# hustvl/LSFA

Measured on AMD Instinct MI355X. Metric: frames/sec/GPU at 1000x600 key_interval=10 (whole-job frames/s), higher is better.
Workload: dtype f32

## Files before the change

### include/lsfa_hip.h

```cpp
#ifndef LSFA_HIP_H_
#define LSFA_HIP_H_

#include <stddef.h>
#include <stdint.h>

#ifdef __cplusplus
extern "C" {
#endif

#define LSFA_OK 0
#define LSFA_EINVAL (-1)
#define LSFA_EWORKSPACE (-2)
#define LSFA_ENOTSUP (-3)

const char* lsfa_last_error(void);
int lsfa_abi_version(void);

int lsfa_psroi_pool_fwd(const float* data, const float* rois,
                        int N, int C, int H, int W, int R,
                        float spatial_scale, int output_dim, int pooled_size, int group_size,
                        float* out, float* mapping_channel, void* stream);

int lsfa_rfcn_head_fwd(const float* cls_map, const float* box_map, const float* rois,
                       int N, int H, int W, int R, int ncls, int nbox,
// ... 76 lines not shown
                               double im_h, double im_w, double scale,
                               double score_thresh, double nms_thresh, int max_per_image,
                               double* dets, int* counts, int* keep_idx,
                               void* ws, size_t ws_bytes, void* stream);

int lsfa_rpn_softmax_split(const float* logits, int N, int H, int W, int ld, int A, float* cls_prob, float* bbox_pred, void* stream);

int lsfa_bbox_pred_clip(const float* rois, const float* deltas, int R, int nreg,
                        double im_h, double im_w, double scale, double* pred_boxes, void* stream);

int lsfa_deform_im2col(const float* data, const float* offset,
                       int N, int C, int H, int W, int kh, int kw,
                       int pad, int stride, int dilate, int deform_groups,
                       int Ho, int Wo, float* col, void* stream);

int lsfa_deform_im2col_cl(const float* data, const float* offset,
                          int N, int C, int H, int W, int kh, int kw,
                          int pad, int stride, int dilate, int deform_groups,
                          int Ho, int Wo, float* col, void* stream);
int lsfa_deform_im2col_cl_ld(const float* data, const float* offset, int offset_ld,
                             int N, int C, int H, int W, int kh, int kw,
                             int pad, int stride, int dilate, int deform_groups,
                             int Ho, int Wo, float* col, void* stream);

size_t lsfa_conv_nhwc_workspace_bytes(int N, int H, int W, int Cout, int kh, int kw, int stride, int pad, int dil);
int lsfa_conv_nhwc_fwd(const float* x, int N, int H, int W, int Cin, const float* w, const float* bias, int Cout,
                       int kh, int kw, int stride, int pad, int dil, int relu, float* y,
                       void* ws, size_t ws_bytes, void* stream);

int lsfa_conv_nhwc_fused_fwd(const float* x, int N, int H, int W, int Cin, const float* w, const float* bias, int Cout,
                             int kh, int kw, int stride, int pad, int dil, int relu, const float* residual, float* y,
                             float* y2, const float* scale2, const float* shift2,
                             void* ws, size_t ws_bytes, void* stream);

typedef struct lsfa_conv_desc {
  const float* x; int lda; int N, H, W, Cin;
  const void* wfrag; int pieces; int w_exp; const float* amax_in;
  const float* bias; int Cout, kh, kw, stride, pad_h, pad_w, dil;
  int act; int y_nchw; const float* residual; float* y; int ldy;
  float* y2; const float* scale2; const float* shift2;
  unsigned* amax_out; unsigned* status;
  int Ho, Wo, out_H, out_W, out_sy, out_sx;
  int prof_tag;
  int x_nchw;
  const float* in_scale;
  const float* in_shift;
  const float* w_scale;
} lsfa_conv_desc;
size_t lsfa_conv_weight_bytes(int Cout, int kh, int kw, int Cin, int pieces);
int lsfa_conv_weights(const float* w, int Cout, int kh, int kw, int Cin, int pieces, int w_exp, void* wfrag, void* stream);
int lsfa_conv_weights_pc(const float* w, int Cout, int kh, int kw, int Cin, const int* w_exp_pc, void* wfrag, void* stream);
size_t lsfa_conv_workspace_bytes(const lsfa_conv_desc* d);
int lsfa_conv_fwd(const lsfa_conv_desc* d, void* ws, size_t ws_bytes, void* stream);
int lsfa_amax_partial(const float* x, long long n, float* out256, void* stream);
#define LSFA_EOVERFLOW (-4)
int lsfa_status_check(unsigned* status_dev, void* stream);
int lsfa_conv_plan_override(int kernel, int nt, int st, int slices);
int lsfa_conv_order_override(int tile_order, int k_order);
int lsfa_conv_plan_query(const lsfa_conv_desc* d, int* out8);
size_t lsfa_deconv4x4s2_crop_workspace_bytes(int N, int Hi, int Wi, int Cin, int Cout, int Hc, int Wc, int pieces);
int lsfa_deconv4x4s2_crop_fwd(const float* x, int lda, int N, int Hi, int Wi, int Cin, const void* wfrag4, int pieces, int w_exp,
                              const float* amax_in, const float* bias, int Cout, int act, float* y, int ldy, int Hc, int Wc,
                              unsigned* amax_out, unsigned* status, void* ws, size_t ws_bytes, void* stream);

int lsfa_avgpool_nchw(const float* x, int N, int C, int H, int W, int k, float* y, void* stream);
int lsfa_avgpool_nchw_tbl(const float* const* x_table, int N, int C, int H, int W, int k, float* y, void* stream);
int lsfa_image_transform_u8(const unsigned char* im_hwc_bgr, int N, int H, int W, const double* pixel_means_bgr_host, double pixel_scale,
                            float* data_nchw, void* stream);
size_t lsfa_stem_weight_bytes(void);
int lsfa_stem_weights(const float* w_l, void* wfrag, void* stream);
int lsfa_stem_conv7x7s2(const float* x, int N, int H, int W, const float* in_scale, const float* in_shift,
                        const void* wfrag, const float* bias, float* y, void* stream);
int lsfa_maxpool3x3s2_nhwc(const float* x, int N, int H, int W, int C, float* y, float* y2, const float* scale2,
                           const float* shift2, unsigned* amax_out, void* stream);
int lsfa_stem_conv7x7s2_ex(const float* x, int N, int H, int W, const float* in_scale, const float* in_shift,
                           const void* wfrag, const float* bias, const float* accum, int act, float* y, unsigned* amax_out,
                           void* stream);
int lsfa_stem_conv7x7s2_tbl(const float* const* x_table, int N, int H, int W, const float* in_scale, const float* in_shift,
                            const void* wfrag, const float* bias, const float* accum, int act, float* y, unsigned* amax_out, void* stream);

int lsfa_head_conv3x3(const float* x, int lda, int N, int H, int W, int Cin, const float* w, const float* bias, int Cout,
                      float mul, float* y, int out_nchw, int ldy, int c0, void* stream);
int lsfa_upsample_flow(const float* in, int N, int Hi, int Wi, int C, const float* w, const float* bias, int Hc, int Wc,
                       float* out, int ldy, int c0, unsigned* amax_out, void* stream);
int lsfa_avgpool2_nhwc(const float* x, int N, int H, int W, int C, float* y, void* stream);
int lsfa_nchw_to_nhwc(const float* x, int N, int Ctot, int HW, int c0, int C, float* y, unsigned* amax_out, void* stream);

int lsfa_scale_shift_relu(const float* x, const float* scale, const float* shift,
                          int N, int C, int HW, int relu, float* y, void* stream);

int lsfa_scale_shift_leaky(const float* x, const float* scale, const float* shift,
                           int N, int C, int HW, float slope, float* y, void* stream);

int lsfa_scale_shift_relu_cl(const float* x, const float* scale, const float* shift,
                             long long rows, int C, int relu, float* y, void* stream);

size_t lsfa_mv_workspace_bytes(int width, int height);
int lsfa_mv_identity(int* accu, int width, int height, void* stream);
int lsfa_mv_accumulate(const int* mvs, int n_mvs, int max_block_area, const int* accu_old, int* accu_new,
                       int width, int height, void* ws, size_t ws_bytes, void* stream);
int lsfa_mv_field(const int* accu, int width, int height, int* mv, void* stream);
int lsfa_mv_residual(const unsigned char* bgr_cur, const unsigned char* bgr_ref, const int* accu,
                     int width, int height, int* res, void* stream);
int lsfa_transform_mv_res(const void* motion_vector, const void* res_diff, int flags, int H, int W, double im_scale, int h1, int w1,
                          int rcnn_stride, const double* pixel_means_bgr_host, double pixel_scale, float* out_mv, float* out_res,
                          int out_h, int out_w, void* stream);
// ... 52 lines not shown
```

### lsfa_amd/build.py

```python
import os
import subprocess
import sys
from concurrent.futures import ThreadPoolExecutor

HERE = os.path.dirname(os.path.abspath(__file__))
CSRC = os.path.join(HERE, "csrc")
INCLUDE = os.path.join(os.path.dirname(HERE), "include")
OBJ = os.path.join(HERE, "csrc", "_obj")
LIB = os.path.join(HERE, "liblsfa_hip.so")
SOURCES = ["runtime.hip", "warp.hip", "aggregate.hip", "psroi.hip", "nms.hip", "proposal.hip", "detpost.hip", "dcn.hip", "mv.hip", "me.hip", "me_segment.hip", "me_pyramid.hip", "yuv.hip", "conv.hip", "conv_exact.hip", "stem.hip", "flownet.hip", "rpn_head.hip", "fuse.hip"]
HIPCC = os.environ.get("HIPCC", "/opt/rocm/bin/hipcc")
FLAGS = ["--offload-arch=gfx950", "-O3", "-std=c++17", "-fPIC", "-ffp-contract=off", "-fno-fast-math",
         "-Wall", "-Wno-unused-function", "-I", INCLUDE, "-I", CSRC] + os.environ.get("LSFA_HIPCC_EXTRA", "-fno-slp-vectorize -fno-vectorize").split()


def _stale(target, deps):
    if not os.path.exists(target):
        return True
    t = os.path.getmtime(target)
    return any(os.path.getmtime(d) > t for d in deps)


def build_hip(force=False, verbose=False):
    os.makedirs(OBJ, exist_ok=True)
    headers = [os.path.join(CSRC, f) for f in os.listdir(CSRC) if f.endswith(".h")] + \
              [os.path.join(INCLUDE, "lsfa_hip.h")]
    jobs = []
    for src in SOURCES:
        s = os.path.join(CSRC, src)
        o = os.path.join(OBJ, src.replace(".hip", ".o"))
        if force or _stale(o, [s] + headers):
            jobs.append((s, o))

    def cc(job):
        s, o = job
        cmd = [HIPCC] + FLAGS + ["-c", s, "-o", o]
        if verbose:
            print(" ".join(cmd))
        r = subprocess.run(cmd, capture_output=True, text=True)
        if r.returncode != 0:
            raise RuntimeError("hipcc failed for %s:\n%s" % (s, r.stderr))
        return r.stderr

    with ThreadPoolExecutor(max_workers=4) as ex:
        for msg in ex.map(cc, jobs):
            if verbose and msg:
                print(msg)
    objs = [os.path.join(OBJ, s.replace(".hip", ".o")) for s in SOURCES]
    if force or jobs or _stale(LIB, objs):
        cmd = [HIPCC, "--offload-arch=gfx950", "-shared", "-fPIC", "-o", LIB] + objs + ["-Wl,-rpath,/opt/rocm/lib"]
        r = subprocess.run(cmd, capture_output=True, text=True)
        if r.returncode != 0:
            raise RuntimeError("link failed:\n%s" % r.stderr)
    return LIB


if __name__ == "__main__":
    print(build_hip(force="--force" in sys.argv, verbose=True))
```

### lsfa_amd/hip.py

```python
import ctypes
import math
import os
import re

import numpy as np
import torch

from lsfa_amd import build as _build

_HERE = os.path.dirname(os.path.abspath(__file__))
LIB_PATH = os.environ.get("LSFA_HIP_LIBRARY") or os.path.join(_HERE, "liblsfa_hip.so")

OP_NAMES = ["psroi_pool", "rfcn_head", "warp_bilinear", "aggregate", "proposal", "nms", "det_postprocess",
            "deform_im2col", "scale_shift_relu", "conv_nhwc", "stem", "flownet_small", "mv_estimate"]


class LsfaError(RuntimeError):
    pass


_lib = None
_WARP_VARIANTS = {'auto': 0, 'gather': 1, 'staged': 2}

_HEADER = os.path.join(_build.INCLUDE, "lsfa_hip.h")
# ... 1050 lines not shown
        if out is not None:
            out.copy_(y)
            y = out
        if out2 is not None:
            out2.copy_(torch.relu(y * scale2.view(1, -1, 1, 1) + shift2.view(1, -1, 1, 1)))
            return y, out2
        return y
    want2 = out2 is not None
    if act == 2:
        y = conv_nhwc(x, sw.w_kc, bias, sw.kh, sw.kw, stride, pad, dil, relu=False, out=None, residual=residual)
        y = torch.where(y > 0, y, y * 0.1)
        if out is not None:
            out.copy_(y)
            y = out
        return y
    r = conv_nhwc(x, sw.w_kc, bias, sw.kh, sw.kw, stride, pad, dil, relu=(act == 1), out=out, residual=residual,
                  out2=out2 if want2 else None, scale2=scale2 if want2 else None, shift2=shift2 if want2 else None)
    return r


@_on_tensor_device
def conv_split(x, sw, bias=None, stride=1, pad=0, dil=1, relu=False, out=None, residual=None, out2=None, scale2=None,
               shift2=None, nchw=False, act=None, amax_in=None, amax_out=None, status=None, x_nchw=False, in_scale=None, in_shift=None):
    x = _f32c(x, "x")
    if x_nchw:
        N, Ctot, H, W = x.shape
        Cin = sw.cin
        if Ctot < Cin or (sw.kh, sw.kw, stride, pad, dil) != (1, 1, 1, 0, 1):
            raise LsfaError("conv_split: x_nchw needs a 1x1 / stride 1 / pad 0 convolution on at least %d channels" % Cin)
    else:
        N, H, W, Cin = x.shape
        Ctot = Cin
    if Cin != sw.cin:
        raise LsfaError("conv_split: input has %d channels, the weight %d" % (Cin, sw.cin))
    Cout, kh, kw = sw.cout, sw.kh, sw.kw
    Ho, Wo = (H + 2 * pad - dil * (kh - 1) - 1) // stride + 1, (W + 2 * pad - dil * (kw - 1) - 1) // stride + 1
    if out is None:
        out = torch.empty((N, Cout, Ho, Wo) if nchw else (N, Ho, Wo, Cout), device=x.device, dtype=torch.float32)
    for name, t in (("out", out), ("residual", residual), ("out2", out2)):
        if t is not None and (t.numel() != N * Ho * Wo * Cout or not t.is_contiguous() or t.dtype != torch.float32):
            raise LsfaError("conv_split: %s must be a contiguous float32 tensor of %d elements" % (name, N * Ho * Wo * Cout))
    if sw.pieces == 0:
        return _conv_exact(x, sw, bias, stride, pad, dil, (1 if relu else 0) if act is None else act, out, residual, out2, scale2, shift2, nchw,
                           x_nchw, in_scale, in_shift)
    if amax_in is None and sw.pieces == 2:
        amax_in = amax_partial(x)
    _count_conv(N, Ho, Wo, sw.real_cout, sw.real_cin, kh, kw, sw.pieces)
    _conv_launch("lsfa_conv_fwd", x, sw, N, H, W, out.data_ptr(), lda=Ctot, ldy=Cout, bias=bias, stride=stride, pad=(pad, pad), dil=dil,
                 act=(1 if relu else 0) if act is None else act, nchw=nchw, residual=residual, out2=out2, scale2=scale2, shift2=shift2,
                 amax_in=amax_in, amax_out=amax_out, status=status, x_nchw=x_nchw, in_scale=in_scale, in_shift=in_shift)
    return out if out2 is None else (out, out2)


@_on_tensor_device
def conv_split_view(x, sw, bias, out, stride=1, pad=(0, 0), dil=1, act=0, cin=None, c0=0, grid=None, place=None, amax_in=None,
                    amax_out=None, status=None, cin0=0):
    x = _f32c(x, "x")
    if not (out.is_contiguous() and out.dtype == torch.float32 and out.dim() == 4):
        raise LsfaError("conv_split_view: out must be a contiguous float32 (N, H, W, C) tensor")
    N, H, W, L = x.shape
    cin = sw.cin if cin is None else cin
    if cin != sw.cin or L < cin0 + cin or cin0 < 0 or cin0 % 4:
        raise LsfaError("conv_split_view: the weight has %d input channels, x offers [%d, %d) (of %d)" % (sw.cin, cin0, cin0 + cin, L))
    if c0 < 0 or c0 + sw.cout > out.shape[3] or out.shape[0] != N:
        raise LsfaError("conv_split_view: channels [%d, %d) do not fit out %s" % (c0, c0 + sw.cout, tuple(out.shape)))
    kh, kw = sw.kh, sw.kw
    Hc, Wc = (H + 2 * pad[0] - dil * (kh - 1) - 1) // stride + 1, (W + 2 * pad[1] - dil * (kw - 1) - 1) // stride + 1
    Ho, Wo = grid if grid is not None else (Hc, Wc)
    y0, x0, sy, sx = place if place is not None else (0, 0, 1, 1)
    Hout, Wout, Lout = out.shape[1], out.shape[2], out.shape[3]
    if y0 + (Ho - 1) * sy >= Hout or x0 + (Wo - 1) * sx >= Wout:
        raise LsfaError("conv_split_view: a %dx%d grid placed at (%d,%d) step (%d,%d) leaves out %s" % (Ho, Wo, y0, x0, sy, sx, tuple(out.shape)))
    if sw.pieces == 0:
        if grid is not None or place is not None or (Ho, Wo) != (Hout, Wout):
            raise LsfaError("conv_split_view: the exact-fp32 mode takes whole output grids only")
        xin = x if (L == cin and cin0 == 0) else x[..., cin0:cin0 + cin].contiguous()
        y = _conv_exact(xin, sw, bias, stride, pad[0], dil, act, None, None, None, None, None, False, False, None, None) if pad[0] == pad[1] else None
        if y is None:
            raise LsfaError("conv_split_view: the exact-fp32 mode needs pad_h == pad_w")
        out[..., c0:c0 + sw.cout] = y
        return out
    if amax_in is None and sw.pieces == 2:
        amax_in = amax_partial(x)
    first = out.data_ptr() + 4 * ((y0 * Wout + x0) * Lout + c0)
    view = place is not None or (Ho, Wo) != (Hout, Wout)
    _count_conv(N, Ho, Wo, sw.real_cout, sw.real_cin, kh, kw, sw.pieces)
    _conv_launch("lsfa_conv_fwd (view)", x, sw, N, H, W, first, x_offset=4 * cin0, lda=L, ldy=Lout, bias=bias, stride=stride, pad=pad, dil=dil, act=act,
                 amax_in=amax_in, amax_out=amax_out, status=status, grid=(Ho, Wo), view=(Hout if view else 0, Wout, sy, sx), prof_tag=1)
    return out


class PhaseWeights(list):
    """The four phase weights of a Deconvolution(4x4, stride 2) as SplitWeight views of ONE allocation (`frag4`)."""


def deconv_phase_weights(wt, cin_pad=None, pieces=None):
    cin, cout = int(wt.shape[0]), int(wt.shape[1])
    cpad = int(cin_pad or cin)
    pieces = int(DEFAULT_PIECES if pieces is None else pieces)
    if pieces == 0:
        pieces = 3
    per = lib().lsfa_conv_weight_bytes(cout, 2, 2, cpad, pieces)
    if per == 0:
        raise LsfaError("deconv_phase_weights: Cin=%d must be a multiple of 32 and Cout=%d of 64" % (cpad, cout))
    frag4 = torch.empty(4 * per, dtype=torch.uint8, device=wt.device)
    out = PhaseWeights()
# ... 491 lines not shown
```

### lsfa_amd/symbols/resnet_v1_101_flownet_rfcn.py

```python
import os as _os

import numpy as np
import torch

from lsfa_amd import hip
from lsfa_amd.symbols import params as P

BN_EPS = 2e-5
_FP32_PIECES = int(_os.environ.get('LSFA_CONV_PIECES', '2'))


class TestSymbol(object):

    def __init__(self, kind, cfg):
        assert kind in ('key', 'cur', 'batch')
        self.kind = kind
        self.cfg = cfg
        self.arg_spec, self.aux_spec = {'key': P.key_symbol_spec, 'cur': P.cur_symbol_spec,
                                        'batch': P.batch_symbol_spec}[kind](cfg)
        if kind == 'batch':
            self.data_names = ['data_key', 'data_other', 'im_info']
        else:
            self.data_names = ['data', 'im_info', 'data_key', 'data_key_old', 'motion_vector', 'res_diff',
                               'feat_key_old', 'feat_key']
# ... 161 lines not shown
                d = dict(stage=si, unit=u, bn1=(dev(s1), dev(t1)), dcn=P.is_dcn_unit(si, u, add_dcn),
                         w1=split(fold(arg[p + 'conv1_weight'], s2)), b1=dev(t2), b2=dev(t3), w3=split(arg[p + 'conv3_weight']))
                if u == 1:
                    d['sc'] = split(arg[p + 'sc_weight'])
                if d['dcn']:
                    ow, ob = dev(arg[p + 'conv2_offset_weight']), dev(arg[p + 'conv2_offset_bias'])
                    co = ow.shape[0]
                    wp, bp = _pad_rows(ow, ob, -(-co // 64) * 64)
                    d['off'], d['off_b'] = hip.SplitWeight(wp, real_cout=co, pieces=pieces), bp
                    w2t = dev(w2)
                    d['w2'] = hip.SplitWeight(w2t.permute(0, 2, 3, 1).reshape(w2t.shape[0], -1, 1, 1).contiguous(), pieces=pieces)
                else:
                    d['w2'] = split(w2)
                self.units.append(d)
        self.bn1 = None
        if tail:
            s, t = bn(prefix + 'bn1')
            self.bn1 = (dev(s), dev(t))


CUR_CHANNELS_LAST = _os.environ.get('LSFA_CUR_NCHW') != '1'


class _Slots(object):

    def __init__(self, rows, device, enabled):
        self.rows, self.device, self.enabled, self.t, self.n = rows, device, enabled, None, 0

    def begin(self):
        if self.enabled:
            self.t, self.n = hip.amax_slots(self.rows, self.device), 0
        return self

    def new(self):
        if not self.enabled:
            return None
        if self.n >= self.rows:
            raise hip.LsfaError("amax slots: section needs more than %d rows" % self.rows)
        self.n += 1
        return self.t[self.n - 1]


class Executor(object):

    def __init__(self, sym, arg_params, aux_params, device, dtype, pieces=None):
        self.sym, self.cfg = sym, sym.cfg
        self.device = torch.device(device)
        self.cdtype = dtype
        if dtype not in (torch.float32, torch.bfloat16):
            raise ValueError("Executor: dtype must be torch.float32 or torch.bfloat16")
        self.pieces = (_FP32_PIECES if pieces is None else int(pieces)) if dtype == torch.float32 else 1
        self.flow_pieces = self.pieces
        self.taps = None
        self.status = hip.new_status(self.device)
        self.input_activation_at_cut = _os.environ.get('LSFA_INPUT_ACT_AT_CUT', '1') == '1'
        self.input_activation_min_bytes = int(float(_os.environ.get('LSFA_INPUT_ACT_MIN_MB', '48')) * (1 << 20))
        cfg = self.cfg
        arg = {k: np.asarray(v, dtype=np.float32) for k, v in arg_params.items()}
        aux = {k: np.asarray(v, dtype=np.float32) for k, v in aux_params.items()}
        for k, shp in sym.arg_spec.items():
            if k not in arg:
                raise KeyError(k + ' not initialized')
            if tuple(arg[k].shape) != tuple(shp):
                raise ValueError('shape inconsistent for %s inferred %s provided %s' % (k, shp, arg[k].shape))
        dev, f32 = self.device, torch.float32
        A = cfg.network.NUM_ANCHORS
        std = np.tile(np.asarray(cfg.network.ANCHOR_STDS, np.float32), A)
        mean = np.tile(np.asarray(cfg.network.ANCHOR_MEANS, np.float32), A)
        wb, bb = arg['rpn_bbox_pred_weight'].reshape(4 * A, 512), arg['rpn_bbox_pred_bias']
        if cfg.network.NORMALIZE_RPN:
            wb, bb = wb * std[:, None], bb * std + mean
        w64, b64 = np.zeros((64, 512, 1, 1), np.float32), np.zeros(64, np.float32)
        w64[:6 * A, :, 0, 0] = np.concatenate([arg['rpn_cls_score_weight'].reshape(2 * A, 512), wb], 0)
        b64[:6 * A] = np.concatenate([arg['rpn_cls_score_bias'], bb], 0)
        self.rpn_sw = hip.SplitWeight(_t(w64, dev, f32), real_cout=6 * A, pieces=3 if self.pieces == 2 else self.pieces)
        self.rpn_b = _t(b64, dev, f32)
        self.n_cls_ch = arg['rfcn_cls_weight'].shape[0]
        G = 7
        self.ncls = self.n_cls_ch // (G * G)
        self.nbox = arg['rfcn_bbox_weight'].shape[0] // (G * G)
        wc = arg['rfcn_cls_weight'].reshape(self.ncls, G * G, 512)
        wx = arg['rfcn_bbox_weight'].reshape(self.nbox, G * G, 512)
        w_ps = np.concatenate([wc, wx], 0).transpose(1, 0, 2).reshape(-1, 512)
        b_ps = np.concatenate([arg['rfcn_cls_bias'].reshape(self.ncls, G * G), arg['rfcn_bbox_bias'].reshape(self.nbox, G * G)], 0).T.reshape(-1)
        self.ps_ld = -(-w_ps.shape[0] // 64) * 64
        wp, bp = _pad_rows(_t(w_ps.reshape(-1, 512, 1, 1), dev, f32), _t(b_ps, dev, f32), self.ps_ld)
        self.rfcn_sw, self.rfcn_b_ps = hip.SplitWeight(wp, real_cout=w_ps.shape[0], pieces=self.pieces), bp
        self.proposal = hip.ProposalOp(feature_stride=cfg.network.RPN_FEAT_STRIDE, scales=cfg.network.ANCHOR_SCALES,
                                       ratios=cfg.network.ANCHOR_RATIOS, rpn_pre_nms_top_n=cfg.TEST.RPN_PRE_NMS_TOP_N,
                                       rpn_post_nms_top_n=cfg.TEST.RPN_POST_NMS_TOP_N, threshold=cfg.TEST.RPN_NMS_THRESH,
                                       rpn_min_size=cfg.TEST.RPN_MIN_SIZE)
        two = self.pieces == 2
        small_rows = 16 if cfg.network.small_net_stride == 4 else 32
        self._slots = {'backbone': _Slots(128, dev, two), 'small': _Slots(small_rows, dev, two), 'agg': _Slots(8, dev, two), 'flow': _Slots(16, dev, two),
                       'heads': _Slots(2, dev, two), 'fuse': _Slots(8, dev, two)}
        W = lambda name: _t(arg[name], dev, f32)
        self.fuse_type, self.warp_bn, self.cur_scale = None, None, None
        if sym.kind in ('key', 'batch'):
            self.net = _ResNetWeights(arg, aux, '', 4, cfg.network.add_dcn, True, dev, self.pieces)
            self.feat_w, self.feat_b = hip.SplitWeight(W('feat_conv_3x3_weight'), pieces=self.pieces), W('feat_conv_3x3_bias')
            self._flownet_prepare({k: _t(v, dev, f32) for k, v in arg.items()
                                   if k.startswith(('flow_conv1', 'conv', 'Convolution', 'deconv', 'upsample_flow')) and 'stage' not in k
                                   and not k.startswith('conv0')})
            if sym.kind == 'batch':
                pass
            elif cfg.network.add_Nq_net:
                w2, b2 = _pad_rows(W('Nq_conv2_weight'), W('Nq_conv2_bias'), 64)
                w3, b3 = _pad_rows(W('Nq_conv3_weight'), W('Nq_conv3_bias'), 64, 64)
                self.nq = [(hip.SplitWeight(W('Nq_conv1_weight'), pieces=self.pieces), W('Nq_conv1_bias')),
# ... 23 lines not shown
        def bn_fold(name):
            g, b = arg[name + '_gamma'].astype(np.float64), arg[name + '_beta'].astype(np.float64)
            m, v = aux[name + '_moving_mean'].astype(np.float64), aux[name + '_moving_var'].astype(np.float64)
            sc = g / np.sqrt(v + BN_EPS)
            return sc, b - m * sc

        def last_conv(name):
            w, b = arg[name + '_weight'].astype(np.float64), arg[name + '_bias'].astype(np.float64)
            if bn:
                sc, sh = bn_fold('cur_feat_bn')
                w, b = w * sc.reshape(-1, 1, 1, 1), b * sc + sh
            return split(w), dev_t(b)

        self.cur_scale = (split(arg['cur_scale_weight']), dev_t(arg['cur_scale_bias'])) if net.small_net_scale_before_fuse else None
        if bn:
            sc, sh = bn_fold('warp_conv_feat_bn')
            self.warp_bn = (dev_t(sc), dev_t(sh))
        if fuse == 'add':
            self.fuse_w, self.fuse_b = last_conv('fuse_reduce_add')
        elif fuse == 'addv2':
            self.fuse_c1 = (split(arg['fuse_reduce_add_conv1_weight']), dev_t(arg['fuse_reduce_add_conv1_bias']))
            self.fuse_w, self.fuse_b = last_conv('fuse_reduce_add_conv2')
        else:
            self.fuse_c1 = (split(arg['fuse_reduce_c1_weight']), dev_t(arg['fuse_reduce_c1_bias']))
        if fuse in ('concat', 'concatv1'):
            self.fuse_c2 = (split(arg['fuse_reduce_c2_weight']), dev_t(arg['fuse_reduce_c2_bias']))
            wr = arg['fuse_reduce_weight']
            self.fuse_r_warp, self.fuse_r_cur, self.fuse_r_b = split(wr[:, :512]), split(wr[:, 512:]), dev_t(arg['fuse_reduce_bias'])
        if fuse in ('concatv1', 'concatv2'):
            w1, w2 = arg['s_feat_conv1_weight'], arg['s_feat_conv2_weight']
            self.gate = (dev_t(w1.reshape(w1.shape[0], -1)), dev_t(arg['s_feat_conv1_bias']), dev_t(w2.reshape(w2.shape[0], -1)),
                         dev_t(arg['s_feat_conv2_bias']))

    @property
    def small_net_channels(self):
        if not self.cfg.network.add_small_net:
            return self.cfg.network.DFF_FEAT_DIM
        return 512 if self.fuse_type in ('concat', 'concatv1') else 1024

    def _tap(self, name, x):
        if self.taps is not None:
            self.taps[name] = x

    def check_status(self):
        hip.check_status(self.status)

    def _conv(self, x, sw, bias=None, stride=1, pad=0, dil=1, act=0, amax_in=None, amax_out=None, **kw):
        if sw.pieces != 2:
            amax_in = amax_out = None
        elif amax_in is None:
            amax_in = hip.amax_partial(x)
        return hip.conv_split(x, sw, bias, stride, pad, dil, act=act, amax_in=amax_in, amax_out=amax_out, status=self.status, **kw)

    def _resnet(self, x, net, stages, section):
        S = self._slots[section].begin()
        units = [u for u in net.units if u['stage'] <= stages]
        if net.conv0_exact is not None:
            if isinstance(x, hip.ImageTable):
                x = x.materialize()
            xa = (x * net.bn_data[0].view(1, 3, 1, 1) + net.bn_data[1].view(1, 3, 1, 1)).permute(0, 2, 3, 1)
            xh = torch.zeros(tuple(xa.shape[:3]) + (32,), device=x.device, dtype=torch.float32)
            xh[..., :3] = xa
            y = hip.conv_split(xh, net.conv0_exact, net.conv0_b, 2, 3, 1, act=1)
        else:
            y = hip.stem_conv(x, net.conv0_w_l, net.conv0_b, net.bn_data[0], net.bn_data[1])
        am_a = S.new()
        x4, a = hip.maxpool3x3s2_nhwc(y, scale2=units[0]['bn1'][0], shift2=units[0]['bn1'][1], amax_out=am_a)
        dilate = 1
        pre = None
        for ui, u in enumerate(units):
            first = u['unit'] == 1
            stride = 2 if (first and u['stage'] in (2, 3)) else 1
            ud = dilate
            if first and u['stage'] == 4:
                dilate = dilate * 2
            am_c1, am_c2, am_n = S.new(), S.new(), S.new()
            if pre is None:
                c1 = self._conv(a, u['w1'], u['b1'], act=1, amax_in=am_a, amax_out=am_c1)
            else:
                c1 = self._conv(a, u['w1'], u['b1'], act=1, amax_in=am_a, amax_out=am_c1, in_scale=pre[0], in_shift=pre[1])
            if u['dcn']:
                off = self._conv(c1, u['off'], u['off_b'], 1, ud, ud, amax_in=am_c1)
                col = hip.deform_im2col_cl(c1, off, 3, 3, ud, 1, ud, P.NUM_DEFORMABLE_GROUP)
                c2 = self._conv(col.view(c1.shape[0], c1.shape[1], c1.shape[2], -1), u['w2'], u['b2'], act=1, amax_in=am_c1, amax_out=am_c2)
            else:
                c2 = None
            if first and pre is not None:
                sc = self._conv(a, u['sc'], None, stride, amax_in=am_a, in_scale=pre[0], in_shift=pre[1])
            else:
                sc = self._conv(a, u['sc'], None, stride, amax_in=am_a) if first else x4
            if c2 is None:
                c2 = self._conv(c1, u['w2'], u['b2'], stride, ud, ud, act=1, amax_in=am_c1, amax_out=am_c2)
            nxt = units[ui + 1]['bn1'] if ui + 1 < len(units) else net.bn1
            lone = self.input_activation_at_cut and ui + 1 < len(units) and u['w1'].pieces != 3 and \
                sc.numel() * 4 >= self.input_activation_min_bytes
            pre = None
            if nxt is not None and lone:
                if u['w3'].pieces == 2:
                    x4 = self._conv(c2, u['w3'], None, amax_in=am_c2, amax_out=am_n, out=sc, residual=sc, scale2=nxt[0], shift2=nxt[1])
                else:
                    x4 = self._conv(c2, u['w3'], None, out=sc, residual=sc)
                a, pre = x4, nxt
            elif nxt is not None:
                x4, a = self._conv(c2, u['w3'], None, amax_in=am_c2, amax_out=am_n, out=sc, residual=sc, out2=torch.empty_like(sc),
                                   scale2=nxt[0], shift2=nxt[1])
            else:
                x4, a = self._conv(c2, u['w3'], None, amax_in=am_c2, amax_out=am_n, out=sc, residual=sc), None
            am_a = am_n
        return (a if a is not None else x4), am_a

    def _backbone(self, data):
        a, am = self._resnet(data, self.net, 4, 'backbone')
        return self._conv(a, self.feat_w, self.feat_b, 1, 6, 6, act=1, amax_in=am, nchw=True)

    def _flownet_prepare(self, fw):
        dev, pc = self.device, self.flow_pieces
        own = {}
        w1 = fw['flow_conv1_weight']
        own['c1_cur'] = hip.stem_weight_layout(w1[:, 0:3].contiguous())
        own['c1_ref'] = hip.stem_weight_layout(w1[:, 3:6].contiguous())
        own['in_scale'] = torch.full((3,), 1.0 / 255.0, device=dev)
        own['in_shift'] = torch.zeros(3, device=dev)
        for name in ('conv2', 'conv3', 'conv3_1', 'conv4', 'conv4_1', 'conv5', 'conv5_1', 'conv6', 'conv6_1'):
            own[name] = hip.SplitWeight(fw[name + '_weight'], pieces=pc)

        def pad32(c):
            return -(-c // 32) * 32
        for name in ('deconv5', 'deconv4', 'deconv3', 'deconv2'):
            wt = fw[name + '_weight']
            own[name] = hip.deconv_phase_weights(wt, cin_pad=pad32(wt.shape[0]), pieces=pc)
        ws = fw['Convolution5_scale_weight']
        wsp, _ = _pad_rows(ws, None, ws.shape[0], pad32(ws.shape[1]))
        own['scale'] = hip.SplitWeight(wsp, real_cin=ws.shape[1], pieces=pc)
        for name in ('Convolution1', 'Convolution2', 'Convolution3', 'Convolution4', 'Convolution5'):
            own[name] = fw[name + '_weight'].permute(0, 2, 3, 1).contiguous()
        self._flow_own, self.flow = own, fw

    def _flownet(self, img_cur, img_ref):
        o, fw, dev = self._flow_own, self.flow, self.device
        LEAKY = 2
        N = img_cur.shape[0]
        st = self.status
        S = self._slots['flow'].begin()

        def cmap(h, w, c):
            return hip.zeros_f32((N, h, w, -(-c // 32) * 32), dev)

        def out_hw(h, w, k, stride, pad):
            return (h + 2 * pad - k) // stride + 1, (w + 2 * pad - k) // stride + 1

        def conv(x, am_x, name, stride, pad, out=None, am_out=None, cin=None):
            sw = o[name]
            h, w = out_hw(x.shape[1], x.shape[2], sw.kh, stride, pad)
            if out is None:
                out, am_out = torch.empty((N, h, w, sw.cout), device=dev, dtype=torch.float32), S.new()
            hip.conv_split_view(x, sw, fw[name + '_bias'], out, stride=stride, pad=(pad, pad), act=LEAKY, cin=cin, amax_in=am_x,
                                amax_out=am_out, status=st)
            return out, am_out

        def deconv(x, am_x, name, out, am_out, c0):
            hip.deconv4x4s2_crop(x, o[name], fw[name + '_bias'], out, c0=c0, act=LEAKY, amax_in=am_x, amax_out=am_out, status=st)
# ... 288 lines not shown
```

Baseline: 3829.

## Fuse residual-block 1x1 expand conv with next block's 1x1 reduce conv

```diff
diff --git a/include/lsfa_hip.h b/include/lsfa_hip.h
--- a/include/lsfa_hip.h
+++ b/include/lsfa_hip.h
@@ -152,6 +152,11 @@
 int lsfa_conv_weights_pc(const float* w, int Cout, int kh, int kw, int Cin, const int* w_exp_pc, void* wfrag, void* stream);
 size_t lsfa_conv_workspace_bytes(const lsfa_conv_desc* d);
 int lsfa_conv_fwd(const lsfa_conv_desc* d, void* ws, size_t ws_bytes, void* stream);
+int lsfa_conv_pair_fwd(const float* x, int ldx, int N, int H, int W, int Cm, const float* amax_in, const void* w3frag,
+                       const float* w3_scale, int pieces3, int C, const float* residual, float* y, int ldy, const float* scale2,
+                       const float* shift2, const void* w1frag, const float* w1_scale, int pieces1, int Cn, const float* bias,
+                       float* z, int ldz, int stride, int y_nchw, unsigned* amax_out_sum, unsigned* amax_out_z, unsigned* status,
+                       void* stream);
 int lsfa_amax_partial(const float* x, long long n, float* out256, void* stream);
 #define LSFA_EOVERFLOW (-4)
 int lsfa_status_check(unsigned* status_dev, void* stream);
diff --git a/lsfa_amd/build.py b/lsfa_amd/build.py
--- a/lsfa_amd/build.py
+++ b/lsfa_amd/build.py
@@ -8,7 +8,7 @@
 INCLUDE = os.path.join(os.path.dirname(HERE), "include")
 OBJ = os.path.join(HERE, "csrc", "_obj")
 LIB = os.path.join(HERE, "liblsfa_hip.so")
-SOURCES = ["runtime.hip", "warp.hip", "aggregate.hip", "psroi.hip", "nms.hip", "proposal.hip", "detpost.hip", "dcn.hip", "mv.hip", "me.hip", "me_segment.hip", "me_pyramid.hip", "yuv.hip", "conv.hip", "conv_exact.hip", "stem.hip", "flownet.hip", "rpn_head.hip", "fuse.hip"]
+SOURCES = ["runtime.hip", "warp.hip", "aggregate.hip", "psroi.hip", "nms.hip", "proposal.hip", "detpost.hip", "dcn.hip", "mv.hip", "me.hip", "me_segment.hip", "me_pyramid.hip", "yuv.hip", "conv.hip", "conv_pair.hip", "conv_exact.hip", "stem.hip", "flownet.hip", "rpn_head.hip", "fuse.hip"]
 HIPCC = os.environ.get("HIPCC", "/opt/rocm/bin/hipcc")
 FLAGS = ["--offload-arch=gfx950", "-O3", "-std=c++17", "-fPIC", "-ffp-contract=off", "-fno-fast-math",
          "-Wall", "-Wno-unused-function", "-I", INCLUDE, "-I", CSRC] + os.environ.get("LSFA_HIPCC_EXTRA", "-fno-slp-vectorize -fno-vectorize").split()
diff --git a/lsfa_amd/csrc/conv_pair.hip b/lsfa_amd/csrc/conv_pair.hip
--- /dev/null
+++ b/lsfa_amd/csrc/conv_pair.hip
@@ -0,0 +1,52 @@
+#include "common.h"
+
+#include "conv_pair_kernel.h"
+
+using namespace lsfa;
+
+namespace {
+struct PairKernel { int cm, cn; void (*fn)(convsplit::PairArgs); };
+const PairKernel kPairKernels[] = {{64, 64, convsplit::conv_pair_kernel<2, 2>},
+                                   {64, 128, convsplit::conv_pair_kernel<2, 4>},
+                                   {128, 64, convsplit::conv_pair_kernel<4, 2>},
+                                   {128, 128, convsplit::conv_pair_kernel<4, 4>}};
+}
+
+extern "C" int lsfa_conv_pair_fwd(const float* x, int ldx, int N, int H, int W, int Cm, const float* amax_in, const void* w3frag,
+                                  const float* w3_scale, int pieces3, int C, const float* residual, float* y, int ldy, const float* scale2,
+                                  const float* shift2, const void* w1frag, const float* w1_scale, int pieces1, int Cn, const float* bias,
+                                  float* z, int ldz, int stride, int y_nchw, unsigned* amax_out_sum, unsigned* amax_out_z, unsigned* status,
+                                  void* stream) {
+  const char* who = "lsfa_conv_pair_fwd";
+  LSFA_REQUIRE(N > 0 && H > 0 && W > 0 && Cm > 0 && C > 0 && Cn > 0, "%s: bad shape", who);
+  if (pieces3 != 2 || pieces1 != 2) {
+    set_error("%s: both weights must be cut into two fp16 pieces (pieces %d / %d)", who, pieces3, pieces1);
+    return LSFA_ENOTSUP;
+  }
+  if (C != 4 * Cm || (Cm != 64 && Cm != 128) || (Cn != 64 && Cn != 128)) {
+    set_error("%s: Cm=%d and Cn=%d must be 64 or 128 and C=%d must be 4 Cm", who, Cm, Cn, C);
+    return LSFA_ENOTSUP;
+  }
+  if (ldx != Cm || ldy != C || ldz != Cn || y_nchw || stride != 1) {
+    set_error("%s: dense channels-last maps at stride 1 only (ldx %d, ldy %d, ldz %d, y_nchw %d, stride %d)", who, ldx, ldy, ldz, y_nchw, stride);
+    return LSFA_ENOTSUP;
+  }
+  LSFA_REQUIRE(x && amax_in && w3frag && w3_scale && residual && y && scale2 && shift2 && w1frag && w1_scale && z, "%s: NULL argument", who);
+  LSFA_REQUIRE((((uintptr_t)x | (uintptr_t)residual | (uintptr_t)y | (uintptr_t)z | (uintptr_t)scale2 | (uintptr_t)shift2 | (uintptr_t)bias) & 15) == 0,
+               "%s: operands must be 16-byte aligned", who);
+  LSFA_REQUIRE((const void*)z != (const void*)y && (const void*)z != (const void*)x && (const void*)y != (const void*)x, "%s: x, y and z must not alias", who);
+  const long P = (long)N * H * W;
+  LSFA_REQUIRE((P + 128) * C < (1L << 31), "%s: tensor too large", who);
+  convsplit::PairArgs a = {};
+  a.x = x; a.amax = amax_in;
+  a.w3 = (const uint4*)w3frag; a.w3scale = w3_scale; a.res = residual; a.y = y; a.scale2 = scale2; a.shift2 = shift2;
+  a.w1 = (const uint4*)w1frag; a.w1scale = w1_scale; a.bias = bias; a.z = z;
+  a.amax_sum = amax_out_sum; a.amax_z = amax_out_z; a.status = status;
+  a.P = (int)P;
+  hipStream_t s = (hipStream_t)stream;
+  ProfScope prof(LSFA_OP_CONV, s);
+  for (const PairKernel& k : kPairKernels)
+    if (k.cm == Cm && k.cn == Cn) hipLaunchKernelGGL(k.fn, dim3((unsigned)((P + 127) / 128)), dim3(convsplit::kThreads), 0, s, a);
+  LSFA_LAUNCH_CHECK(who);
+  return LSFA_OK;
+}
diff --git a/lsfa_amd/csrc/conv_pair_kernel.h b/lsfa_amd/csrc/conv_pair_kernel.h
--- /dev/null
+++ b/lsfa_amd/csrc/conv_pair_kernel.h
@@ -0,0 +1,248 @@
+#pragma once
+#include "conv_ring_kernel.h"
+
+namespace lsfa {
+namespace convsplit {
+
+struct PairArgs {
+  const float* x; const float* amax;
+  const uint4* w3; const float* w3scale; const float* res; float* y; const float* scale2; const float* shift2;
+  const uint4* w1; const float* w1scale; const float* bias; float* z;
+  unsigned* amax_sum; unsigned* amax_z; unsigned* status;
+  int P;
+};
+
+constexpr int kPairStage = 512;
+
+constexpr int pair_groups(int KM, int KN) { return (KM == 2 && KN == 2) ? 1 : 2; }
+
+template <int KM, int KN>
+__device__ __forceinline__ void pair_issue(uint4* R0, uint4* R1, const PairArgs& a, int j, int i, int wave, int lane) {
+  constexpr int kW3 = 2 * KM;
+  const uint4* src;
+  if (i < kW3) {
+    const int c = pair_groups(KM, KN) == 1 ? i >> 1 : i % KM, h = pair_groups(KM, KN) == 1 ? i & 1 : i / KM;
+    src = a.w3 + (size_t)(c * (4 * KM) + 4 * j + 2 * h) * 256;
+  } else {
+    const int h = (i - kW3) / 4, c = (i - kW3) % 4;
+    src = a.w1 + (size_t)((4 * j + c) * KN + 2 * h) * 256;
+  }
+  src += wave * 128 + lane;
+  uint4* dst = ((i & 1) ? R1 : R0) + wave * 128;
+  __builtin_amdgcn_global_load_lds(src, dst, 16, 0, 0);
+  __builtin_amdgcn_global_load_lds(src + 64, dst + 64, 16, 0, 0);
+}
+
+template <int NA>
+__device__ __forceinline__ void pair_mma(const uint4* B, const Cut& p, f32x16 (&acc)[NA], int h) {
+  uint4 b[2][2];
+#pragma unroll
+  for (int s = 0; s < 2; ++s) {
+#pragma unroll
+    for (int tt = 0; tt < 2; ++tt)
+#pragma unroll
+      for (int q = 0; q < 2; ++q) b[tt][q] = B[((tt * 2 + s) * 2 + q) * 64];
+#pragma unroll
+    for (int tt = 0; tt < 2; ++tt) acc[2 * h + tt] = mma_pc<2>(s ? p.s1 : p.s0, b[tt][0], b[tt][1], b[tt][1], acc[2 * h + tt]);
+  }
+}
+
+__device__ __forceinline__ Cut pair_cut(const uint4* A, const int (&frag)[4], float s) {
+  const uint4 r0 = A[frag[0]], r1 = A[frag[1]], r2 = A[frag[2]], r3 = A[frag[3]];
+  Cut n;
+  n.s0 = cut8<2>(as_f4(r0), as_f4(r1), s);
+  n.s1 = cut8<2>(as_f4(r2), as_f4(r3), s);
+  return n;
+}
+
+__device__ __forceinline__ void pair_sync() {
+  __builtin_amdgcn_s_waitcnt(0x0070);
+  __builtin_amdgcn_s_barrier();
+}
+
+template <int KM, int KN>
+static __global__ __launch_bounds__(kThreads, (KM == 4 && KN == 4) ? 1 : 2) void conv_pair_kernel(PairArgs a) {
+  constexpr int Cm = 32 * KM, C = 4 * Cm, Cn = 32 * KN;
+  constexpr int kW3 = 2 * KM, kSB = 2 * KM + 2 * KN;
+  constexpr int kGroups = pair_groups(KM, KN), kGroupTiles = 4 / kGroups, kGroupStages = kW3 / kGroups;
+  static_assert((KM == 2 || KM == 4) && (KN == 2 || KN == 4), "Cm and Cn are 64 or 128");
+  __shared__ __attribute__((aligned(16))) uint4 R0[kPairStage];
+  __shared__ __attribute__((aligned(16))) uint4 R1[kPairStage];
+  __shared__ __attribute__((aligned(16))) uint4 S[4][1024];
+  const int tid = threadIdx.x, lane = tid & 63;
+  const int wave = __builtin_amdgcn_readfirstlane(tid >> 6);
+  const int P = a.P;
+  const int m0 = blockIdx.x * kWgPix + wave * kWavePix;
+  uint4* Sw = &S[wave][0];
+  float* Tf = reinterpret_cast<float*>(Sw);
+
+  const uint32_t* am = reinterpret_cast<const uint32_t*>(a.amax);
+  uint32_t mi = max(max(am[lane] & 0x7FFFFFFFu, am[lane + 64] & 0x7FFFFFFFu), max(am[lane + 128] & 0x7FFFFFFFu, am[lane + 192] & 0x7FFFFFFFu));
+#pragma unroll
+  for (int c = 0; c < KM; ++c)
+#pragma unroll
+    for (int i = 0; i < 4; ++i) {
+      const int pix = m0 + 8 * i + (lane >> 3);
+      const int piece = (lane & 7) ^ ((4 * i + (lane >> 4)) & 7);
+      const float* src = pix < P ? a.x + (pix * Cm + c * kChunk + 4 * piece) : g_zero_block;
+      __builtin_amdgcn_global_load_lds(reinterpret_cast<const uint4*>(src), Sw + c * 256 + i * 64, 16, 0, 0);
+    }
+  pair_issue<KM, KN>(R0, R1, a, 0, 0, wave, lane);
+#pragma unroll
+  for (int d = 32; d >= 1; d >>= 1) mi = max(mi, (uint32_t)__shfl_xor((int)mi, d, 64));
+  const int ei = (int)((mi >> 23) & 255u);
+  if (ei == 255 && a.status && lane == 0) atomicOr(a.status, 2u);
+  const int s_in = 13 - ((ei == 0 || ei == 255) ? 0 : __builtin_amdgcn_readfirstlane(ei - 127));
+  const float a_scale = ldexpf(1.f, s_in), inv_in = ldexpf(1.f, -s_in);
+
+  int frag[4];
+  {
+    const int r = lane & 31, h = lane >> 5, sw = (r >> 1) & 7;
+#pragma unroll
+    for (int k = 0; k < 4; ++k) frag[k] = r * 8 + ((4 * h + k) ^ sw);
+  }
+  const int c4 = (lane & 7) * 4;
+  int base[4], rowf[4];
+  bool ok[4];
+#pragma unroll
+  for (int k = 0; k < 4; ++k) {
+    const int row = 8 * k + (lane >> 3), p = m0 + row;
+    ok[k] = p < P;
+    base[k] = ok[k] ? p : 0;
+    rowf[k] = row * 32 + (((lane & 7) ^ ((row >> 1) & 7)) << 2);
+  }
+  const int accl = 128 * (lane >> 5) + (((((lane & 31) >> 2) ^ ((lane >> 5) << 1)) << 2) | (lane & 3));
+#define PAIR_ACCF(r) ((((r) & 3) + 8 * ((r) >> 2)) * 32 + (accl ^ (((((r) & 3) >> 1) | ((((r) >> 2) & 1) << 2)) << 2)))
+
+  __builtin_amdgcn_s_waitcnt(0x0F70);
+  Cut pc[KM];
+#pragma unroll
+  for (int c = 0; c < KM; ++c) pc[c] = pair_cut(Sw + c * 256, frag, a_scale);
+
+  f32x16 sum1[KN];
+#pragma unroll
+  for (int t = 0; t < KN; ++t)
+#pragma unroll
+    for (int r = 0; r < 16; ++r) sum1[t][r] = 0.f;
+  float mx_sum = 0.f, nf_sum = 0.f;
+
+#pragma unroll 1
+  for (int j = 0; j < KM; ++j) {
+    float mx = 0.f;
+#pragma unroll
+    for (int gq = 0; gq < kGroups; ++gq) {
+      f32x16 acc3[kGroupTiles];
+      float os3[kGroupTiles];
+#pragma unroll
+      for (int t = 0; t < kGroupTiles; ++t)
+#pragma unroll
+        for (int r = 0; r < 16; ++r) acc3[t][r] = 0.f;
+#pragma unroll
+      for (int q = 0; q < kGroupStages; ++q) {
+        const int i = gq * kGroupStages + q;
+        pair_sync();
+        pair_issue<KM, KN>(R0, R1, a, j, i + 1, wave, lane);
+        if (q == 0) {
+#pragma unroll
+          for (int tq = 0; tq < kGroupTiles; ++tq) os3[tq] = a.w3scale[(unsigned)(j * 128 + (gq * kGroupTiles + tq) * 32 + (lane & 31))] * inv_in;
+        }
+        pair_mma<kGroupTiles>(((i & 1) ? R1 : R0) + lane, pc[kGroups == 1 ? q >> 1 : q], acc3, kGroups == 1 ? q & 1 : 0);
+      }
+#pragma unroll
+      for (int tq = 0; tq < kGroupTiles; ++tq)
+#pragma unroll
+        for (int r = 0; r < 16; ++r) Tf[(gq * kGroupTiles + tq) * 1024 + PAIR_ACCF(r)] = (0.f + acc3[tq][r]) * os3[tq];
+      float4 rr[4][kGroupTiles];
+#pragma unroll
+      for (int k = 0; k < 4; ++k)
+#pragma unroll
+        for (int tq = 0; tq < kGroupTiles; ++tq)
+          rr[k][tq] = *reinterpret_cast<const float4*>(a.res + (unsigned)(base[k] * C + j * 128 + (gq * kGroupTiles + tq) * 32 + c4));
+#pragma unroll
+      for (int tq = 0; tq < kGroupTiles; ++tq) {
+        const int t = gq * kGroupTiles + tq;
+        const float4 s2 = *reinterpret_cast<const float4*>(a.scale2 + (unsigned)(j * 128 + t * 32 + c4));
+        const float4 h2 = *reinterpret_cast<const float4*>(a.shift2 + (unsigned)(j * 128 + t * 32 + c4));
+#pragma unroll
+        for (int k = 0; k < 4; ++k) {
+          float4* slot = reinterpret_cast<float4*>(&Tf[t * 1024 + rowf[k]]);
+          float4 o = *slot;
+          float4 w = make_float4(0.f, 0.f, 0.f, 0.f);
+          if (ok[k]) {
+            o.x = o.x + rr[k][tq].x; o.y = o.y + rr[k][tq].y; o.z = o.z + rr[k][tq].z; o.w = o.w + rr[k][tq].w;
+            nf_sum = nf_sum + fabsf(o.x); nf_sum = nf_sum + fabsf(o.y); nf_sum = nf_sum + fabsf(o.z); nf_sum = nf_sum + fabsf(o.w);
+            *reinterpret_cast<float4*>(a.y + (unsigned)(base[k] * C + j * 128 + t * 32 + c4)) = o;
+            w.x = fmaxf(o.x * s2.x + h2.x, 0.f); w.y = fmaxf(o.y * s2.y + h2.y, 0.f);
+            w.z = fmaxf(o.z * s2.z + h2.z, 0.f); w.w = fmaxf(o.w * s2.w + h2.w, 0.f);
+            mx = fmaxf(fmaxf(mx, fmaxf(w.x, w.y)), fmaxf(w.z, w.w));
+          }
+          *slot = w;
+        }
+      }
+    }
+    mx_sum = fmaxf(mx_sum, mx);
+    uint32_t mb = __float_as_uint(mx);
+#pragma unroll
+    for (int d = 32; d >= 1; d >>= 1) mb = max(mb, (uint32_t)__shfl_xor((int)mb, d, 64));
+    const int eb = __builtin_amdgcn_readfirstlane((int)((mb >> 23) & 255u));
+    const int s_b = (eb == 0 || eb == 255) ? 0 : min(13 - (eb - 127), 100);
+    const float b_scale = ldexpf(1.f, s_b), inv_b = ldexpf(1.f, -s_b);
+
+#pragma unroll
+    for (int h = 0; h < KN / 2; ++h) {
+      f32x16 acc1[2];
+#pragma unroll
+      for (int t = 0; t < 2; ++t)
+#pragma unroll
+        for (int r = 0; r < 16; ++r) acc1[t][r] = 0.f;
+#pragma unroll
+      for (int c = 0; c < 4; ++c) {
+        const int i = kW3 + 4 * h + c;
+        pair_sync();
+        if (i + 1 < kSB) pair_issue<KM, KN>(R0, R1, a, j, i + 1, wave, lane);
+        else if (j + 1 < KM) pair_issue<KM, KN>(R0, R1, a, j + 1, 0, wave, lane);
+        const Cut ap = pair_cut(Sw + c * 256, frag, b_scale);
+        pair_mma<2>(((i & 1) ? R1 : R0) + lane, ap, acc1, 0);
+      }
+#pragma unroll
+      for (int t = 0; t < 2; ++t) {
+        const float os1 = a.w1scale[(unsigned)((2 * h + t) * 32 + (lane & 31))] * inv_b;
+#pragma unroll
+        for (int r = 0; r < 16; ++r) sum1[2 * h + t][r] = sum1[2 * h + t][r] + acc1[t][r] * os1;
+      }
+    }
+  }
+  {
+    uint32_t m = __float_as_uint(mx_sum);
+    if ((__float_as_uint(nf_sum) & 0x7F800000u) == 0x7F800000u) m = 0x7FC00000u;
+    publish_amax(m, a.amax_sum, a.status, blockIdx.x * 4 + wave);
+  }
+#pragma unroll
+  for (int t = 0; t < KN; ++t)
+#pragma unroll
+    for (int r = 0; r < 16; ++r) Tf[t * 1024 + PAIR_ACCF(r)] = sum1[t][r];
+  float4 bb[KN];
+#pragma unroll
+  for (int t = 0; t < KN; ++t) bb[t] = a.bias ? *reinterpret_cast<const float4*>(a.bias + (unsigned)(t * 32 + c4)) : make_float4(0.f, 0.f, 0.f, 0.f);
+  float mx = 0.f, nf = 0.f;
+#pragma unroll
+  for (int k = 0; k < 4; ++k)
+#pragma unroll
+    for (int t = 0; t < KN; ++t) {
+      float4 o = *reinterpret_cast<const float4*>(&Tf[t * 1024 + rowf[k]]);
+      if (!ok[k]) continue;
+      o.x = o.x + bb[t].x; o.y = o.y + bb[t].y; o.z = o.z + bb[t].z; o.w = o.w + bb[t].w;
+      nf = nf + fabsf(o.x); nf = nf + fabsf(o.y); nf = nf + fabsf(o.z); nf = nf + fabsf(o.w);
+      o.x = fmaxf(o.x, 0.f); o.y = fmaxf(o.y, 0.f); o.z = fmaxf(o.z, 0.f); o.w = fmaxf(o.w, 0.f);
+      *reinterpret_cast<float4*>(a.z + (unsigned)(base[k] * Cn + t * 32 + c4)) = o;
+      mx = fmaxf(fmaxf(mx, fmaxf(o.x, o.y)), fmaxf(o.z, o.w));
+    }
+  uint32_t m = __float_as_uint(mx);
+  if ((__float_as_uint(nf) & 0x7F800000u) == 0x7F800000u) m = 0x7FC00000u;
+  publish_amax(m, a.amax_z, a.status, blockIdx.x * 4 + wave);
+}
+
+#undef PAIR_ACCF
+
+}
+}
diff --git a/lsfa_amd/hip.py b/lsfa_amd/hip.py
--- a/lsfa_amd/hip.py
+++ b/lsfa_amd/hip.py
@@ -1126,6 +1126,51 @@
     return out if out2 is None else (out, out2)
 
 
+def _pair_kernel_name(cm, cn):
+    return "conv_pair_kernel<%d, %d>" % (cm // 32, cn // 32)
+
+
+@_on_tensor_device
+def conv_pair(x, sw3, residual, scale2, shift2, sw1, bias=None, out=None, out_z=None, amax_in=None, amax_out_sum=None, amax_out_z=None,
+              status=None, stride=1, nchw=False):
+    if x.dim() != 4 or x.dtype != torch.float32:
+        raise LsfaError("conv_pair: x must be a (N, H, W, Cm) float32 tensor")
+    N, H, W, Cm = x.shape
+    C, Cn = sw3.cout, sw1.cout
+    if (sw3.kh, sw3.kw, sw1.kh, sw1.kw) != (1, 1, 1, 1) or sw3.cin != Cm or sw1.cin != C:
+        raise LsfaError("conv_pair: two 1x1 convolutions Cm=%d -> C -> Cn, not %dx%d %d -> %d and %dx%d %d -> %d"
+                        % (Cm, sw3.kh, sw3.kw, sw3.cin, C, sw1.kh, sw1.kw, sw1.cin, Cn))
+    if getattr(sw3, 'w_scale', None) is None or getattr(sw1, 'w_scale', None) is None:
+        if sw3.pieces == 2 and sw1.pieces == 2:
+            raise LsfaError("conv_pair: the weights must carry per-channel scales (SplitWeight(per_channel_scale=True))")
+    if amax_in is None:
+        amax_in = amax_partial(_f32c(x, "x"))
+    if out is None:
+        out = torch.empty((N, H, W, C), device=x.device, dtype=torch.float32)
+    if out_z is None:
+        out_z = torch.empty((N, H, W, Cn), device=x.device, dtype=torch.float32)
+    for name, t, c in (("out", out, C), ("residual", residual, C), ("out_z", out_z, Cn)):
+        if t is None or t.numel() != N * H * W * c or t.dtype != torch.float32:
+            raise LsfaError("conv_pair: %s must be a float32 tensor of %d elements" % (name, N * H * W * c))
+    ldx = x.stride(2) if x.stride(3) == 1 else 0
+    ldy = out.stride(-2) if out.stride(-1) == 1 and out.dim() == 4 else C
+    ldz = out_z.stride(-2) if out_z.stride(-1) == 1 and out_z.dim() == 4 else Cn
+    if not (residual.is_contiguous() and scale2.is_contiguous() and shift2.is_contiguous()):
+        raise LsfaError("conv_pair: residual, scale2 and shift2 must be contiguous")
+    if _conv_flops["count"] and sw3.pieces == 2 and sw1.pieces == 2:
+        P = N * H * W
+        f = 2.0 * P * (Cm * C + C * Cn)
+        _conv_flops["flops"] += f
+        _conv_flops["launches"] += 1
+        _conv_flops["flops_three_products"] += f
+        _count_conv_launch(_pair_kernel_name(Cm, Cn), f, 4.0 * P * (Cm + 2 * C + Cn) + 4.0 * (Cm * C + C * Cn))
+    _check(lib().lsfa_conv_pair_fwd(x.data_ptr(), ldx, N, H, W, Cm, _ptr(amax_in), _ptr(sw3.frag), _ptr(getattr(sw3, 'w_scale', None)), sw3.pieces, C,
+                                    _ptr(residual), out.data_ptr(), ldy, _ptr(scale2), _ptr(shift2), _ptr(sw1.frag),
+                                    _ptr(getattr(sw1, 'w_scale', None)), sw1.pieces, Cn, _ptr(bias), out_z.data_ptr(), ldz, int(stride), int(nchw),
+                                    _ptr(amax_out_sum), _ptr(amax_out_z), _ptr(status), _stream()), "lsfa_conv_pair_fwd")
+    return out, out_z
+
+
 @_on_tensor_device
 def conv_split_view(x, sw, bias, out, stride=1, pad=(0, 0), dil=1, act=0, cin=None, c0=0, grid=None, place=None, amax_in=None,
                     amax_out=None, status=None, cin0=0):
diff --git a/lsfa_amd/symbols/resnet_v1_101_flownet_rfcn.py b/lsfa_amd/symbols/resnet_v1_101_flownet_rfcn.py
--- a/lsfa_amd/symbols/resnet_v1_101_flownet_rfcn.py
+++ b/lsfa_amd/symbols/resnet_v1_101_flownet_rfcn.py
@@ -237,9 +237,13 @@
         self.pieces = (_FP32_PIECES if pieces is None else int(pieces)) if dtype == torch.float32 else 1
         self.flow_pieces = self.pieces
         self.taps = None
+        self.stage_taps = None
         self.status = hip.new_status(self.device)
         self.input_activation_at_cut = _os.environ.get('LSFA_INPUT_ACT_AT_CUT', '1') == '1'
         self.input_activation_min_bytes = int(float(_os.environ.get('LSFA_INPUT_ACT_MIN_MB', '48')) * (1 << 20))
+        self.pair_1x1 = int(_os.environ.get('LSFA_PAIR_1X1', '1'))
+        if self.pair_1x1 not in (0, 1, 2):
+            raise ValueError("LSFA_PAIR_1X1 must be 0, 1 or 2")
         cfg = self.cfg
         arg = {k: np.asarray(v, dtype=np.float32) for k, v in arg_params.items()}
         aux = {k: np.asarray(v, dtype=np.float32) for k, v in aux_params.items()}
@@ -369,6 +373,11 @@
             amax_in = hip.amax_partial(x)
         return hip.conv_split(x, sw, bias, stride, pad, dil, act=act, amax_in=amax_in, amax_out=amax_out, status=self.status, **kw)
 
+    @staticmethod
+    def _pairable(w3, w1):
+        return w3.pieces == 2 and w1.pieces == 2 and getattr(w3, 'w_scale', None) is not None and getattr(w1, 'w_scale', None) is not None and \
+            (w3.kh, w3.kw, w1.kh, w1.kw) == (1, 1, 1, 1) and w3.cin in (64, 128) and w3.cout == 4 * w3.cin and w1.cin == w3.cout and w1.cout in (64, 128)
+
     def _resnet(self, x, net, stages, section):
         S = self._slots[section].begin()
         units = [u for u in net.units if u['stage'] <= stages]
@@ -385,14 +394,17 @@
         x4, a = hip.maxpool3x3s2_nhwc(y, scale2=units[0]['bn1'][0], shift2=units[0]['bn1'][1], amax_out=am_a)
         dilate = 1
         pre = None
+        carry = None
         for ui, u in enumerate(units):
             first = u['unit'] == 1
             stride = 2 if (first and u['stage'] in (2, 3)) else 1
             ud = dilate
             if first and u['stage'] == 4:
                 dilate = dilate * 2
-            am_c1, am_c2, am_n = S.new(), S.new(), S.new()
-            if pre is None:
+            am_c1, am_c2, am_n = (carry[1] if carry is not None else S.new()), S.new(), S.new()
+            if carry is not None:
+                c1, carry = carry[0], None
+            elif pre is None:
                 c1 = self._conv(a, u['w1'], u['b1'], act=1, amax_in=am_a, amax_out=am_c1)
             else:
                 c1 = self._conv(a, u['w1'], u['b1'], act=1, amax_in=am_a, amax_out=am_c1, in_scale=pre[0], in_shift=pre[1])
@@ -412,7 +424,13 @@
             lone = self.input_activation_at_cut and ui + 1 < len(units) and u['w1'].pieces != 3 and \
                 sc.numel() * 4 >= self.input_activation_min_bytes
             pre = None
-            if nxt is not None and lone:
+            nu = units[ui + 1] if ui + 1 < len(units) else None
+            if nu is not None and u['stage'] <= self.pair_1x1 and self._pairable(u['w3'], nu['w1']):
+                am_z = S.new()
+                x4, z = hip.conv_pair(c2, u['w3'], sc, nxt[0], nxt[1], nu['w1'], nu['b1'], out=sc, amax_in=am_c2, amax_out_sum=am_n,
+                                      amax_out_z=am_z, status=self.status)
+                a, pre, carry = x4, nxt, (z, am_z)
+            elif nxt is not None and lone:
                 if u['w3'].pieces == 2:
                     x4 = self._conv(c2, u['w3'], None, amax_in=am_c2, amax_out=am_n, out=sc, residual=sc, scale2=nxt[0], shift2=nxt[1])
                 else:
@@ -424,6 +442,8 @@
             else:
                 x4, a = self._conv(c2, u['w3'], None, amax_in=am_c2, amax_out=am_n, out=sc, residual=sc), None
             am_a = am_n
+            if self.stage_taps is not None and (nu is None or nu['stage'] != u['stage']):
+                self.stage_taps['%s_stage%d' % (section, u['stage'])] = x4
         return (a if a is not None else x4), am_a
 
     def _backbone(self, data):
```

Result: faster. 3894, median of 6 (+1.7%).
